# LordTARN1SHED/Image-Restoration-for-Road-Sign-Recognition-in-Autonomous-Driving

Measured on AMD Instinct MI355X. Metric: images/sec ResUNet fwd+bwd (64x64 GTSRB batch) at 1/2/4/8 MI355X; PSNR parity, higher is better.
Workload: dtype bf16; 1 GPU; cfg3: ResUNet unified train step (dynamic distortion + ToTensor, fwd + L1 + 0.1*VGG16[:16] perceptual + bwd + AdamW), 14_train_unified_advanced.py; global_batch=512, per_gpu_batch=512, parallelism=dp1, hip_graph=True

## Files before the change

image-restoration-for-road-sign-recognition-in-autonomous-driving_amd/csrc/common.h:

```cpp
#pragma once
#include <hip/hip_runtime.h>
#include <stdint.h>
#include <stdlib.h>

#include <type_traits>

#include "../../include/roadrestore.h"

typedef __bf16 bf16x8 __attribute__((ext_vector_type(8)));
typedef float f32x4 __attribute__((ext_vector_type(4)));
typedef short s16x4 __attribute__((ext_vector_type(4)));
typedef unsigned short u16;
typedef u16 u16x4 __attribute__((ext_vector_type(4)));
typedef u16 u16x8 __attribute__((ext_vector_type(8)));

#define LDS_PTR(p) ((__attribute__((address_space(3))) void *)(p))

struct bf16_t {
  u16 v;
};

__device__ __forceinline__ float bf16_to_f32(u16 b) {
  return __uint_as_float(((uint32_t)b) << 16);
}
__device__ __forceinline__ u16 f32_to_bf16(float f) {
  return __builtin_bit_cast(u16, static_cast<__bf16>(f));
}

template <typename T> struct Elt;
template <> struct Elt<float> {
  static constexpr int size = 4;
  static constexpr int dtype = RR_F32;
  __device__ __forceinline__ static float load(const float *p, long long i) { return p[i]; }
  __device__ __forceinline__ static void store(float *p, long long i, float v) { p[i] = v; }
  __device__ __forceinline__ static float round(float v) { return v; }
};
template <> struct Elt<bf16_t> {
  static constexpr int size = 2;
  static constexpr int dtype = RR_BF16;
  __device__ __forceinline__ static float load(const bf16_t *p, long long i) {
    return bf16_to_f32(p[i].v);
  }
  __device__ __forceinline__ static void store(bf16_t *p, long long i, float v) {
    p[i].v = f32_to_bf16(v);
  }
  __device__ __forceinline__ static float round(float v) { return bf16_to_f32(f32_to_bf16(v)); }
};

template <typename T> __device__ __forceinline__ f32x4 load4(const T *p);
template <> __device__ __forceinline__ f32x4 load4<float>(const float *p) {
  return *reinterpret_cast<const f32x4 *>(p);
}
template <> __device__ __forceinline__ f32x4 load4<bf16_t>(const bf16_t *p) {
  u16x4 r = *reinterpret_cast<const u16x4 *>(p);
  f32x4 o;
  o[0] = bf16_to_f32(r[0]); o[1] = bf16_to_f32(r[1]);
  o[2] = bf16_to_f32(r[2]); o[3] = bf16_to_f32(r[3]);
  return o;
}
template <typename T> __device__ __forceinline__ void store4(T *p, f32x4 v);
template <> __device__ __forceinline__ void store4<float>(float *p, f32x4 v) {
  *reinterpret_cast<f32x4 *>(p) = v;
}
template <> __device__ __forceinline__ void store4<bf16_t>(bf16_t *p, f32x4 v) {
  u16x4 r;
  r[0] = f32_to_bf16(v[0]); r[1] = f32_to_bf16(v[1]);
  r[2] = f32_to_bf16(v[2]); r[3] = f32_to_bf16(v[3]);
  *reinterpret_cast<u16x4 *>(p) = r;
}

template <typename T> __device__ __forceinline__ void load8(const T *p, f32x4 &a, f32x4 &b);
template <> __device__ __forceinline__ void load8<float>(const float *p, f32x4 &a, f32x4 &b) {
  a = *reinterpret_cast<const f32x4 *>(p);
  b = *reinterpret_cast<const f32x4 *>(p + 4);
}
template <> __device__ __forceinline__ void load8<bf16_t>(const bf16_t *p, f32x4 &a, f32x4 &b) {
  const uint4 r = *reinterpret_cast<const uint4 *>(p);
  a[0] = __uint_as_float(r.x << 16); a[1] = __uint_as_float(r.x & 0xffff0000u);
  a[2] = __uint_as_float(r.y << 16); a[3] = __uint_as_float(r.y & 0xffff0000u);
  b[0] = __uint_as_float(r.z << 16); b[1] = __uint_as_float(r.z & 0xffff0000u);
  b[2] = __uint_as_float(r.w << 16); b[3] = __uint_as_float(r.w & 0xffff0000u);
}

template <typename T> __device__ __forceinline__ void store8(T *p, f32x4 a, f32x4 b);
template <> __device__ __forceinline__ void store8<float>(float *p, f32x4 a, f32x4 b) {
  *reinterpret_cast<f32x4 *>(p) = a;
  *reinterpret_cast<f32x4 *>(p + 4) = b;
}
template <> __device__ __forceinline__ void store8<bf16_t>(bf16_t *p, f32x4 a, f32x4 b) {
  u16x8 r;
  r[0] = f32_to_bf16(a[0]); r[1] = f32_to_bf16(a[1]); r[2] = f32_to_bf16(a[2]); r[3] = f32_to_bf16(a[3]);
  r[4] = f32_to_bf16(b[0]); r[5] = f32_to_bf16(b[1]); r[6] = f32_to_bf16(b[2]); r[7] = f32_to_bf16(b[3]);
  *reinterpret_cast<u16x8 *>(p) = r;
}

template <int CTRL> __device__ __forceinline__ float dpp_f(float v) {
  return __int_as_float(__builtin_amdgcn_update_dpp(0, __float_as_int(v), CTRL, 0xF, 0xF, false));
}
constexpr int DPP_XOR1 = 0xB1, DPP_XOR2 = 0x4E, DPP_HALF_MIRROR = 0x141, DPP_MIRROR = 0x140;
__device__ __forceinline__ float row16_sum(float v) {
  v += dpp_f<DPP_XOR1>(v);
  v += dpp_f<DPP_XOR2>(v);
  v += dpp_f<DPP_HALF_MIRROR>(v);
  v += dpp_f<DPP_MIRROR>(v);
  return v;
}
__device__ __forceinline__ float max_xor1(float v) { return fmaxf(v, dpp_f<DPP_XOR1>(v)); }
__device__ __forceinline__ uint32_t xor1_u32(uint32_t v) {
  return (uint32_t)__builtin_amdgcn_update_dpp(0, (int)v, DPP_XOR1, 0xF, 0xF, false);
}
__device__ __forceinline__ float pool4_first_max(float v0, float v1, float v2, float v3, uint32_t &id) {
  float m = v0;
  uint32_t k = 0;
  bool t = !(v1 <= m) & (m == m);
  m = t ? v1 : m; k = t ? 1u : k;
  t = !(v2 <= m) & (m == m);
  m = t ? v2 : m; k = t ? 2u : k;
  t = !(v3 <= m) & (m == m);
  m = t ? v3 : m; k = t ? 3u : k;
  id = k;
  return m;
}

__device__ __forceinline__ float wave_sum(float v) {
#pragma unroll
  for (int o = 32; o > 0; o >>= 1) v += __shfl_xor(v, o, 64);
  return v;
}

#ifdef RR_DRYRUN
extern "C" void rr_dry_launch(const void *kernel, const unsigned *grid3, const unsigned *block3);
template <typename... A> static inline void rr_dry(const void *k, dim3 g, dim3 b, const A &...) {
  const unsigned g3[3] = {g.x, g.y, g.z}, b3[3] = {b.x, b.y, b.z};
  rr_dry_launch(k, g3, b3);
}
#undef hipLaunchKernelGGL
#define hipLaunchKernelGGL(k, g, b, shmem, st, ...) rr_dry((const void *)(k), dim3(g), dim3(b), __VA_ARGS__)
#define RR_LAUNCH_FAILED() false
#else
#define RR_LAUNCH_FAILED() (hipGetLastError() != hipSuccess)
#endif

#define RR_CHECK_LAUNCH()                        \
  do {                                           \
    if (RR_LAUNCH_FAILED()) return RR_ELAUNCH;   \
  } while (0)

static inline bool rr_dtype_ok(int dtype) { return dtype == RR_BF16 || dtype == RR_F32; }
template <int N> using ic = std::integral_constant<int, N>;
template <typename T> struct EltTag { using type = T; };
template <typename F> static inline int rr_dispatch_elt(int dtype, F &&f) {
  if (dtype == RR_BF16) return f(EltTag<bf16_t>{});
  if (dtype == RR_F32) return f(EltTag<float>{});
  return RR_EINVAL;
}
template <int... Vs, typename F> static inline int rr_dispatch_int(int v, F &&f) {
  int r = RR_EINVAL;
  (void)(... || (v == Vs && ((r = f(ic<Vs>{})), true)));
  return r;
}

struct RrPath {
  int stream3 = 1, stream3_strips = 1, stream1 = 1, stream1_minp = 131072;
  int conv3r = 1, conv3r_w64 = 1, conv3r_wg = 0, conv3r_segwg = 0;
  int igemm_halo = 1, swgrad = 1, wgrad_halo = 1, blur_tiled = 1;
  int rdist_tile = 32;
};

static inline RrPath rr_path_read() {
  RrPath r;
  const char *e = getenv("RR_PATH");
  if (!e || !*e) return r;
  static const struct { const char *key; int RrPath::*field; } keys[] = {
      {"stream3", &RrPath::stream3}, {"stream3_strips", &RrPath::stream3_strips},
      {"stream1", &RrPath::stream1}, {"stream1_minp", &RrPath::stream1_minp},
      {"conv3r", &RrPath::conv3r}, {"conv3r_w64", &RrPath::conv3r_w64},
      {"conv3r_wg", &RrPath::conv3r_wg}, {"conv3r_segwg", &RrPath::conv3r_segwg},
      {"igemm_halo", &RrPath::igemm_halo}, {"swgrad", &RrPath::swgrad},
      {"wgrad_halo", &RrPath::wgrad_halo}, {"blur_tiled", &RrPath::blur_tiled},
      {"rdist_tile", &RrPath::rdist_tile}};
  unsigned seen = 0;
  for (const char *p = e; *p;) {
    const char *q = p;
    while (*q && *q != ',') ++q;
    const char *eq = p;
    while (eq < q && *eq != '=') ++eq;
    const char *k0 = p, *k1 = eq, *v0 = eq < q ? eq + 1 : q, *v1 = q;
    while (k0 < k1 && *k0 == ' ') ++k0;
    while (k1 > k0 && k1[-1] == ' ') --k1;
    while (v0 < v1 && *v0 == ' ') ++v0;
    while (v1 > v0 && v1[-1] == ' ') --v1;
    const bool neg = v0 < v1 && *v0 == '-';
    if (v0 < v1 && (*v0 == '-' || *v0 == '+')) ++v0;
    int val = 0;
    bool ok = eq < q && v1 > v0 && v1 - v0 <= 9;
    for (const char *c = v0; ok && c < v1; ++c) {
      ok = *c >= '0' && *c <= '9';
      val = val * 10 + (*c - '0');
    }
    for (unsigned i = 0; ok && i < sizeof keys / sizeof keys[0]; ++i) {
      const size_t kl = __builtin_strlen(keys[i].key);
      if ((size_t)(k1 - k0) != kl || __builtin_memcmp(k0, keys[i].key, kl) != 0) continue;
      if (!(seen >> i & 1)) r.*keys[i].field = neg ? -val : val;
      seen |= 1u << i;
    }
    p = *q ? q + 1 : q;
  }
  return r;
}

static inline int rr_grid_cap(long long want, int cap = 2048) {
  if (want < 1) return 1;
  return (int)(want < cap ? want : cap);
}

static __device__ __attribute__((aligned(16))) const char rr_zero_page[256] = {0};

struct FastDiv {
  uint32_t d, m, s;
};
static inline FastDiv make_fastdiv(uint32_t d) {
  FastDiv f;
  f.d = d;
  uint32_t s = 0;
  while ((1ull << s) < d) ++s;
  f.s = s;
  f.m = (uint32_t)(((1ull << 32) * ((1ull << s) - d)) / d + 1);
  return f;
}
__device__ __forceinline__ uint32_t fdiv(uint32_t n, const FastDiv &f) {
  const uint32_t t = __umulhi(n, f.m);
  return (t + n) >> f.s;
}

template <int NC, int U = (NC == 1 ? 16 : 8), typename T>
__device__ __forceinline__ void rr_fixed_sum(const T *__restrict__ p, long long stride, long long n,
                                             double (&s)[NC]) {
  long long i = 0;
  for (; i + U <= n; i += U) {
    T v[U][NC];
#pragma unroll
    for (int u = 0; u < U; ++u)
#pragma unroll
      for (int k = 0; k < NC; ++k) v[u][k] = p[(i + u) * stride + k];
#pragma unroll
    for (int u = 0; u < U; ++u)
#pragma unroll
      for (int k = 0; k < NC; ++k) s[k] += (double)v[u][k];
  }
  for (; i < n; ++i)
#pragma unroll
    for (int k = 0; k < NC; ++k) s[k] += (double)p[i * stride + k];
}
__device__ __forceinline__ long long rr_trips(long long first, long long end, long long step) {
  return first < end ? (end - first + step - 1) / step : 0;
}

__global__ static void rr_colreduce_kernel(const float *__restrict__ in, int rows, int cols,
                                           int rows_per_chunk, double *__restrict__ out) {
  __shared__ double red[4][64];
  const int tc = threadIdx.x & 63, l = threadIdx.x >> 6;
  const int c = blockIdx.x * 64 + tc;
  const long long r0 = (long long)blockIdx.y * rows_per_chunk;
  const long long r1 = min((long long)rows, r0 + rows_per_chunk);
  double s[1] = {0.0};
  if (c < cols) rr_fixed_sum<1>(in + (r0 + l) * cols + c, 4LL * cols, rr_trips(r0 + l, r1, 4), s);
  red[l][tc] = s[0];
  __syncthreads();
  if (l == 0 && c < cols) out[(long long)blockIdx.y * cols + c] = red[0][tc] + red[1][tc] + red[2][tc] + red[3][tc];
}

static inline int rr_colreduce_chunks(int rows) { return rows < 64 ? (rows < 1 ? 1 : rows) : 64; }
static inline size_t rr_colreduce_bytes(int rows, int cols) {
  return (size_t)rr_colreduce_chunks(rows) * cols * sizeof(double);
}
static inline int rr_colreduce(const float *in, int rows, int cols, double *out, hipStream_t st) {
  const int chunks = rr_colreduce_chunks(rows);
  const int rpc = (rows + chunks - 1) / chunks;
  hipLaunchKernelGGL(rr_colreduce_kernel, dim3((cols + 63) / 64, chunks), dim3(256), 0, st, in, rows,
                     cols, rpc, out);
  return RR_LAUNCH_FAILED() ? -1 : chunks;
}
```

image-restoration-for-road-sign-recognition-in-autonomous-driving_amd/csrc/conv_in.hip:

```cpp
#include "common.h"

namespace {

template <typename T>
__global__ void conv_in_fwd_kernel(int n, int h, int w, int cin, int cout,
                                   const float *__restrict__ x, const float *__restrict__ wt,
                                   const float *__restrict__ b, int act, const float *alpha,
                                   T *__restrict__ y) {
  extern __shared__ __attribute__((aligned(16))) float sw[];
  const int kk = cin * 9;
  for (int i = threadIdx.x; i < kk * cout; i += blockDim.x) {
    const int co = i % cout, j = i / cout;
    sw[i] = wt[(long long)co * kk + j];
  }
  for (int i = threadIdx.x; i < cout; i += blockDim.x) sw[kk * cout + i] = b ? b[i] : 0.f;
  __syncthreads();
  const int G = cout / 4;
  const long long P = (long long)n * h * w;
  const float al = alpha ? alpha[0] : 0.f;
  for (long long id = blockIdx.x * (long long)blockDim.x + threadIdx.x; id < P * G;
       id += (long long)gridDim.x * blockDim.x) {
    const int g = (int)(id % G);
    const long long p = id / G;
    const int ww = (int)(p % w);
    const long long nh = p / w;
    const int hh = (int)(nh % h);
    const int nn = (int)(nh / h);
    f32x4 acc = *reinterpret_cast<const f32x4 *>(sw + kk * cout + g * 4);
    for (int ci = 0; ci < cin; ++ci) {
      const float *xp = x + ((long long)nn * cin + ci) * h * w;
#pragma unroll
      for (int t = 0; t < 9; ++t) {
        const int y2 = hh + t / 3 - 1, x2 = ww + t % 3 - 1;
        if (y2 < 0 || y2 >= h || x2 < 0 || x2 >= w) continue;
        const float v = xp[(long long)y2 * w + x2];
        acc += v * *reinterpret_cast<const f32x4 *>(sw + (ci * 9 + t) * cout + g * 4);
      }
    }
    if (act == 1) {
#pragma unroll
      for (int k = 0; k < 4; ++k) acc[k] = fmaxf(acc[k], 0.f);
    } else if (act == 2) {
#pragma unroll
      for (int k = 0; k < 4; ++k) acc[k] = acc[k] > 0.f ? acc[k] : al * acc[k];
    }
    store4<T>(y + p * cout + g * 4, acc);
  }
}

template <typename T>
__global__ void conv_in_wgrad_kernel(int n, int h, int w, int cin, int cout,
                                     const float *__restrict__ x, const T *__restrict__ dy,
                                     float *__restrict__ part, long long px_per_block) {
  __shared__ __attribute__((aligned(16))) float sdy[64][65];
  __shared__ __attribute__((aligned(16))) float spt[64][32];
  const int kk = cin * 9;
  const long long P = (long long)n * h * w;
  const long long pb = blockIdx.x * px_per_block;
  const long long pe = min(P, pb + px_per_block);
  const int co = threadIdx.x & 63, jg = threadIdx.x >> 6;
  double acc[8] = {0, 0, 0, 0, 0, 0, 0, 0};
  for (long long p0 = pb; p0 < pe; p0 += 64) {
    __syncthreads();
    for (int i = threadIdx.x; i < 64 * 64; i += blockDim.x) {
      const int r = i >> 6, c = i & 63;
      const long long p = p0 + r;
      sdy[r][c] = (p < pe && c < cout) ? Elt<T>::load(dy, p * cout + c) : 0.f;
    }
    for (int i = threadIdx.x; i < 64 * 32; i += blockDim.x) {
      const int r = i >> 5, j = i & 31;
      const long long p = p0 + r;
      float v = 0.f;
      if (p < pe) {
        if (j < kk) {
          const int ci = j / 9, t = j % 9;
          const int ww = (int)(p % w);
          const long long nh = p / w;
          const int hh = (int)(nh % h);
          const int nn = (int)(nh / h);
          const int y2 = hh + t / 3 - 1, x2 = ww + t % 3 - 1;
          if (y2 >= 0 && y2 < h && x2 >= 0 && x2 < w)
            v = x[(((long long)nn * cin + ci) * h + y2) * w + x2];
        } else if (j == kk) {
          v = 1.f;
        }
      }
      spt[r][j] = v;
    }
    __syncthreads();
    if (co < cout) {
      float st[8] = {0.f, 0.f, 0.f, 0.f, 0.f, 0.f, 0.f, 0.f};
#pragma unroll 4
      for (int r = 0; r < 64; ++r) {
        const float d = sdy[r][co];
        const f32x4 a0 = *reinterpret_cast<const f32x4 *>(&spt[r][jg * 8]);
        const f32x4 a1 = *reinterpret_cast<const f32x4 *>(&spt[r][jg * 8 + 4]);
#pragma unroll
        for (int k = 0; k < 4; ++k) { st[k] += d * a0[k]; st[4 + k] += d * a1[k]; }
      }
#pragma unroll
      for (int k = 0; k < 8; ++k) acc[k] += st[k];
    }
  }
  if (co < cout) {
#pragma unroll
    for (int k = 0; k < 8; ++k) part[((long long)blockIdx.x * cout + co) * 32 + jg * 8 + k] = (float)acc[k];
  }
}

constexpr int CIA_NPX = 64;
constexpr int CIA_ROW = CIA_NPX + 8;
constexpr int CIA_XROW = 32 + 8;
template <bool REC>
__global__ __launch_bounds__(256, REC ? 4 : 1) void conv_in_wgrad_act_kernel(
    int n, int h, int w, const float *__restrict__ x, const bf16_t *__restrict__ g,
    const bf16_t *__restrict__ t, int act, const float *__restrict__ alpha,
    float *__restrict__ part, long long ppb) {
  __shared__ __attribute__((aligned(16))) u16 gT[64 * CIA_ROW];
  __shared__ __attribute__((aligned(16))) u16 pT[32 * CIA_ROW];
  __shared__ __attribute__((aligned(16))) u16 pX[REC ? CIA_NPX * CIA_XROW : 8];
  __shared__ float red[256];
  const int tid = threadIdx.x, lane = tid & 63, wv = tid >> 6;
  const long long P = (long long)n * h * w, hw = (long long)h * w;
  const long long p0 = blockIdx.x * ppb, p1 = min(P, p0 + ppb);
  const float al = act == 2 ? alpha[0] : 0.f;
  float sa = 0.f;
  f32x4 acc[2] = {f32x4{0.f, 0.f, 0.f, 0.f}, f32x4{0.f, 0.f, 0.f, 0.f}};
  const int lc = tid & 7, lpp = tid >> 3;
  const int bn = lane & 15, bk = lane >> 4;
  const int sj = tid & 63, sg = tid >> 6;
  uint4 rg[2], rt[2] = {};
  float rp[8];
  auto load_step = [&](long long q0) __attribute__((always_inline)) {
#pragma unroll
    for (int j = 0; j < 2; ++j) {
      const long long p = q0 + 2 * lpp + j;
      const bool ok = p < p1;
      const long long e = (ok ? p : p0) * 64 + lc * 8;
      rg[j] = *reinterpret_cast<const uint4 *>(g + e);
      if constexpr (!REC) rt[j] = *reinterpret_cast<const uint4 *>(t + e);
      if (!ok) rg[j] = uint4{0u, 0u, 0u, 0u};
    }
    const long long p = q0 + sj;
    const bool live = p < p1;
    int img = 0, y = 0, xx0 = 0;
    if (live) {
      img = (int)(p / hw);
      const int rem = (int)(p - img * hw);
      y = rem / w;
      xx0 = rem - y * w;
    }
#pragma unroll
    for (int u = 0; u < 8; ++u) {
      const int r = sg + 4 * u;
      float val = 0.f;
      if (r < 27) {
        const int ci = r / 9, ky = (r % 9) / 3, kx = r % 3;
        const int yy = y + ky - 1, xx = xx0 + kx - 1;
        const bool ok = live && yy >= 0 && yy < h && xx >= 0 && xx < w;
        const float vv = x[ok ? (((long long)img * 3 + ci) * h + yy) * w + xx : 0];
        val = ok ? vv : 0.f;
      } else if (r == 27) {
        val = live ? 1.f : 0.f;
      }
      rp[u] = val;
    }
  };
  auto bf = [](uint32_t word, int hi) { return __uint_as_float(hi ? (word & 0xffff0000u) : (word << 16)); };
  bf16x8 fw = {};
  if constexpr (REC) fw = *reinterpret_cast<const bf16x8 *>(t + (wv * 16 + bn) * 32 + bk * 8);
  if (p0 < p1) load_step(p0);
  for (long long q0 = p0; q0 < p1; q0 += CIA_NPX) {
    if constexpr (REC) {
#pragma unroll
      for (int u = 0; u < 8; ++u) {
        const u16 pv = f32_to_bf16(rp[u]);
        pT[(sg + 4 * u) * CIA_ROW + sj] = pv;
        pX[sj * CIA_XROW + sg + 4 * u] = pv;
      }
      __syncthreads();
#pragma unroll
      for (int nb = 0; nb < 4; ++nb) {
        const bf16x8 fp = *reinterpret_cast<const bf16x8 *>(&pX[(nb * 16 + bn) * CIA_XROW + bk * 8]);
        const f32x4 tv = __builtin_amdgcn_mfma_f32_16x16x32_bf16(fw, fp, f32x4{0.f, 0.f, 0.f, 0.f}, 0, 0, 0);
#pragma unroll
        for (int i = 0; i < 4; ++i) gT[(wv * 16 + 4 * bk + i) * CIA_ROW + nb * 16 + bn] = f32_to_bf16(tv[i]);
      }
      __syncthreads();
    }
    u16 v[2][8];
    uint32_t tpair[8];
    if constexpr (REC) {
#pragma unroll
      for (int k = 0; k < 8; ++k)
        tpair[k] = *reinterpret_cast<const uint32_t *>(&gT[(lc * 8 + k) * CIA_ROW + 2 * lpp]);
    }
#pragma unroll
    for (int j = 0; j < 2; ++j) {
      const uint32_t gw[4] = {rg[j].x, rg[j].y, rg[j].z, rg[j].w};
      const uint32_t tw[4] = {rt[j].x, rt[j].y, rt[j].z, rt[j].w};
#pragma unroll
      for (int k = 0; k < 8; ++k) {
        const float gg = bf(gw[k >> 1], k & 1);
        const float tt = REC ? bf(tpair[k], j) : bf(tw[k >> 1], k & 1);
        const float gp = tt > 0.f ? gg : al * gg;
        sa += tt > 0.f ? 0.f : gg * tt;
        v[j][k] = f32_to_bf16(gp);
      }
    }
#pragma unroll
    for (int k = 0; k < 8; ++k)
      *reinterpret_cast<uint32_t *>(&gT[(lc * 8 + k) * CIA_ROW + 2 * lpp]) =
          (uint32_t)v[0][k] | ((uint32_t)v[1][k] << 16);
    if constexpr (!REC) {
#pragma unroll
      for (int u = 0; u < 8; ++u) pT[(sg + 4 * u) * CIA_ROW + sj] = f32_to_bf16(rp[u]);
    }
    __syncthreads();
    if (q0 + CIA_NPX < p1) load_step(q0 + CIA_NPX);
#pragma unroll
    for (int ks = 0; ks < 2; ++ks) {
      const int px = ks * 32 + bk * 8;
      const bf16x8 fa = *reinterpret_cast<const bf16x8 *>(&gT[(wv * 16 + bn) * CIA_ROW + px]);
#pragma unroll
      for (int nb = 0; nb < 2; ++nb) {
        const bf16x8 fb = *reinterpret_cast<const bf16x8 *>(&pT[(nb * 16 + bn) * CIA_ROW + px]);
        acc[nb] = __builtin_amdgcn_mfma_f32_16x16x32_bf16(fa, fb, acc[nb], 0, 0, 0);
      }
    }
    __syncthreads();
  }
  float *pw = part + (long long)blockIdx.x * (64 * 32 + 32);
#pragma unroll
  for (int nb = 0; nb < 2; ++nb)
#pragma unroll
    for (int i = 0; i < 4; ++i) pw[(wv * 16 + 4 * bk + i) * 32 + nb * 16 + bn] = acc[nb][i];
  red[tid] = sa;
  __syncthreads();
  for (int o = 128; o > 0; o >>= 1) {
    if (tid < o) red[tid] += red[tid + o];
    __syncthreads();
  }
  if (tid < 32) pw[64 * 32 + tid] = tid == 0 ? red[0] : 0.f;
}

__global__ void conv_in_wgrad_act_finalize(int chunks, const double *__restrict__ part, float *dw,
                                           float *db, float *dalpha) {
  const int i = blockIdx.x * blockDim.x + threadIdx.x;
  const int cols = 64 * 32 + 32;
  if (i > 64 * 32) return;
  double sv[1] = {0};
  rr_fixed_sum<1>(part + i, cols, chunks, sv);
  const double s = sv[0];
  if (i == 64 * 32) {
    if (dalpha) dalpha[0] = (float)s;
    return;
  }
  const int co = i / 32, j = i % 32;
  if (j < 27) dw[co * 27 + j] = (float)s;
  else if (j == 27 && db) db[co] = (float)s;
}

__global__ void conv_in_wgrad_finalize(int cout, int kk, int blocks, const double *__restrict__ part,
                                       float *dw, float *db) {
  const int i = blockIdx.x * blockDim.x + threadIdx.x;
  if (i >= cout * 32) return;
  const int co = i / 32, j = i % 32;
  if (j > kk) return;
  double sv[1] = {0};
  rr_fixed_sum<1>(part + i, (long long)cout * 32, blocks, sv);
  const double s = sv[0];
  if (j < kk) dw[(long long)co * kk + j] = (float)s;
  else if (db) db[co] = (float)s;
}

template <typename T>
__global__ void conv_in_dgrad_kernel(int n, int h, int w, int cin, int cout,
                                     const T *__restrict__ dy, const float *__restrict__ wt,
                                     float *__restrict__ dx, int accumulate) {
  extern __shared__ __attribute__((aligned(16))) float sw[];
  const int kk = cin * 9;
  for (int i = threadIdx.x; i < kk * cout; i += blockDim.x) {
    const int co = i % cout, j = i / cout;
    const int t = j / cin, ci = j % cin;
    sw[i] = wt[((long long)co * cin + ci) * 9 + t];
  }
  __syncthreads();
  const long long P = (long long)n * h * w;
  for (long long p = blockIdx.x * (long long)blockDim.x + threadIdx.x; p < P;
       p += (long long)gridDim.x * blockDim.x) {
    const int ww = (int)(p % w);
    const long long nh = p / w;
    const int hh = (int)(nh % h);
    const int nn = (int)(nh / h);
    float acc[4] = {0.f, 0.f, 0.f, 0.f};
    for (int t = 0; t < 9; ++t) {
      const int ky = t / 3, kx = t % 3;
      const int y2 = hh - ky + 1, x2 = ww - kx + 1;
      if (y2 < 0 || y2 >= h || x2 < 0 || x2 >= w) continue;
      const T *dp = dy + (((long long)nn * h + y2) * w + x2) * cout;
      for (int c = 0; c < cout; c += 4) {
        const f32x4 d = load4<T>(dp + c);
        for (int ci = 0; ci < cin && ci < 4; ++ci) {
          const f32x4 wv = *reinterpret_cast<const f32x4 *>(sw + (t * cin + ci) * cout + c);
          acc[ci] += d[0] * wv[0] + d[1] * wv[1] + d[2] * wv[2] + d[3] * wv[3];
        }
      }
    }
    for (int ci = 0; ci < cin && ci < 4; ++ci) {
      const long long o = (((long long)nn * cin + ci) * h + hh) * w + ww;
      dx[o] = accumulate ? dx[o] + acc[ci] : acc[ci];
    }
  }
}

template <typename T>
__global__ void im2col3_kernel(int n, int h, int w, int cin, int kpad, const float *__restrict__ x,
                               T *__restrict__ col) {
  const int G = kpad / 4;
  const long long total = (long long)n * h * w * G;
  const int kk = cin * 9;
  for (long long i = blockIdx.x * (long long)blockDim.x + threadIdx.x; i < total;
       i += (long long)gridDim.x * blockDim.x) {
    const int g = (int)(i % G);
    const long long p = i / G;
    const int ww = (int)(p % w);
    const long long nh = p / w;
    const int hh = (int)(nh % h);
    const int nn = (int)(nh / h);
    f32x4 v;
#pragma unroll
    for (int e = 0; e < 4; ++e) {
      const int j = g * 4 + e;
      float val = 0.f;
      if (j < kk) {
        const int ci = j / 9, t = j - (j / 9) * 9;
        const int y2 = hh + t / 3 - 1, x2 = ww + t % 3 - 1;
        if (y2 >= 0 && y2 < h && x2 >= 0 && x2 < w)
          val = x[(((long long)nn * cin + ci) * h + y2) * w + x2];
      } else if (j == kk) {
        val = 1.f;
      }
      v[e] = val;
    }
    store4<T>(col + p * kpad + g * 4, v);
  }
}

__global__ __launch_bounds__(256) void conv_in_mfma_kernel(int n, int h, int w,
                                                           const float *__restrict__ x,
                                                           const bf16_t *__restrict__ wp, int act,
                                                           const float *__restrict__ alpha,
                                                           bf16_t *__restrict__ y_pre,
                                                           bf16_t *__restrict__ y_act) {
  constexpr int SR = 68;
  __shared__ __attribute__((aligned(16))) float stg[4][32 * SR];
  const int lane = threadIdx.x & 63, wv = threadIdx.x >> 6;
  const long long hw = (long long)h * w;
  const long long P = (long long)n * hw;
  const long long p0 = ((long long)blockIdx.x * 4 + wv) * 64;
  if (p0 >= P) return;
  const int fr = lane & 15, q = lane >> 4;
  bf16x8 fa[4];
#pragma unroll
  for (int mi = 0; mi < 4; ++mi)
    fa[mi] = *reinterpret_cast<const bf16x8 *>(wp + (mi * 16 + fr) * 32 + q * 8);
  const int hwi = h * w;
  int kofs[8], kdy[8], kdx[8];
  bool ktap[8], kone[8];
#pragma unroll
  for (int j = 0; j < 8; ++j) {
    const int k = q * 8 + j;
    const int ci = k / 9, t = k - (k / 9) * 9;
    kdy[j] = t / 3 - 1;
    kdx[j] = t % 3 - 1;
    kofs[j] = ci * hwi + kdy[j] * w + kdx[j];
    ktap[j] = k < 27;
    kone[j] = k == 27;
  }
  const int Pi = (int)P;
  const __amdgpu_buffer_rsrc_t xr = __builtin_amdgcn_make_buffer_rsrc(
      const_cast<float *>(x), 0, (int)(3 * P * 4), 0x00020000);
  const int pw0 = (int)p0;
  f32x4 acc[4][4];
#pragma unroll
  for (int ni = 0; ni < 4; ++ni) {
    const int p = pw0 + ni * 16 + fr;
    const bool live = p < Pi;
    const int pc = live ? p : 0;
    const int nn = pc / hwi, rem = pc - (pc / hwi) * hwi;
    const int yy = rem / w, xx = rem - (rem / w) * w;
    const int base = nn * 3 * hwi + rem;
    bf16x8 fb;
#pragma unroll
    for (int j = 0; j < 8; ++j) {
      const int y2 = yy + kdy[j], x2 = xx + kdx[j];
      const bool ok = ktap[j] && live && (unsigned)y2 < (unsigned)h && (unsigned)x2 < (unsigned)w;
      const float v = __builtin_bit_cast(float, __builtin_amdgcn_raw_buffer_load_b32(
          xr, ok ? (base + kofs[j]) * 4 : 0xffffffff, 0, 0));
      fb[j] = (__bf16)(v + (kone[j] ? 1.f : 0.f));
    }
#pragma unroll
    for (int mi = 0; mi < 4; ++mi)
      acc[mi][ni] = __builtin_amdgcn_mfma_f32_16x16x32_bf16(fa[mi], fb, f32x4{0.f, 0.f, 0.f, 0.f},
                                                           0, 0, 0);
  }
  float *sw = stg[wv];
  const float slope = act == 2 ? alpha[0] : (act == 1 ? 0.f : 1.f);
  const int rows = (int)min(64LL, P - p0);
#pragma unroll
  for (int half = 0; half < 2; ++half) {
    if (half) asm volatile("s_waitcnt lgkmcnt(0)" ::: "memory");
#pragma unroll
    for (int mi = 0; mi < 4; ++mi)
#pragma unroll
      for (int nj = 0; nj < 2; ++nj)
        *reinterpret_cast<f32x4 *>(sw + (nj * 16 + fr) * SR + mi * 16 + q * 4) = acc[mi][half * 2 + nj];
    asm volatile("s_waitcnt lgkmcnt(0)" ::: "memory");
#pragma unroll
    for (int i = 0; i < 4; ++i) {
      const int rl = i * 8 + (lane >> 3), c8 = (lane & 7) * 8;
      const int r = half * 32 + rl;
      if (r < rows) {
        const long long p = p0 + r;
        const f32x4 v0 = *reinterpret_cast<const f32x4 *>(sw + rl * SR + c8);
        const f32x4 v1 = *reinterpret_cast<const f32x4 *>(sw + rl * SR + c8 + 4);
        if (y_pre) store8<bf16_t>(y_pre + p * 64 + c8, v0, v1);
        if (y_act) {
          f32x4 a0, a1;
#pragma unroll
          for (int k = 0; k < 4; ++k) {
            a0[k] = v0[k] > 0.f ? v0[k] : slope * v0[k];
            a1[k] = v1[k] > 0.f ? v1[k] : slope * v1[k];
          }
          store8<bf16_t>(y_act + p * 64 + c8, a0, a1);
        }
      }
    }
  }
}

}

extern "C" int rr_im2col3(int dtype, int n, int h, int w, int cin, int kpad, const float *x,
                          void *col, rr_stream stream) {
  if (!x || !col || cin <= 0 || kpad % 4 || kpad < 9 * cin + 1) return RR_EINVAL;
  const long long total = (long long)n * h * w * (kpad / 4);
  dim3 g(rr_grid_cap((total + 255) / 256, 8192)), b(256);
  hipStream_t st = (hipStream_t)stream;
  return rr_dispatch_elt(dtype, [&](auto tag) {
    using T = typename decltype(tag)::type;
    hipLaunchKernelGGL(im2col3_kernel<T>, g, b, 0, st, n, h, w, cin, kpad, x, (T *)col);
    RR_CHECK_LAUNCH();
    return RR_OK;
  });
}

extern "C" int rr_conv_in_fwd(int dtype, int n, int h, int w, int cin, int cout, const float *x,
                              const float *wt, const float *b, int act, const float *alpha,
                              void *y, rr_stream stream) {
  if (!x || !wt || !y || n <= 0 || h <= 0 || w <= 0 || cin <= 0 || cin > 4 || cout % 4 ||
      cout > 128 || (act == 2 && !alpha))
    return RR_EINVAL;
  const long long work = (long long)n * h * w * (cout / 4);
  const size_t shm = ((size_t)cin * 9 * cout + cout) * sizeof(float);
  dim3 g(rr_grid_cap((work + 255) / 256, 8192)), bl(256);
  hipStream_t st = (hipStream_t)stream;
  return rr_dispatch_elt(dtype, [&](auto tag) {
    using T = typename decltype(tag)::type;
    hipLaunchKernelGGL(conv_in_fwd_kernel<T>, g, bl, shm, st, n, h, w, cin, cout, x, wt, b, act,
                       alpha, (T *)y);
    RR_CHECK_LAUNCH();
    return RR_OK;
  });
}

int rr_colreduce_misc(const float *in, int rows, int cols, double *out, hipStream_t st);
static int conv_in_wgrad_blocks(int n, int h, int w) {
  const long long P = (long long)n * h * w;
  long long b = (P + 2047) / 2048;
  if (b > 1024) b = 1024;
  return (int)(b < 1 ? 1 : b);
}

extern "C" size_t rr_conv_in_wgrad_workspace(int n, int h, int w, int cin, int cout) {
  (void)cin;
  const int blocks = conv_in_wgrad_blocks(n, h, w);
  return (size_t)blocks * cout * 32 * sizeof(float) + rr_colreduce_bytes(blocks, cout * 32);
}

extern "C" int rr_conv_in_wgrad(int dtype, int n, int h, int w, int cin, int cout, const float *x,
                                const void *dy, float *dw, float *db, void *ws, size_t ws_bytes,
                                rr_stream stream) {
  if (!x || !dy || !dw || cin * 9 >= 32 || cout > 64 || cout <= 0) return RR_EINVAL;
  const int blocks = conv_in_wgrad_blocks(n, h, w);
  const size_t pbytes = (size_t)blocks * cout * 32 * sizeof(float);
  if (!ws || ws_bytes < pbytes + rr_colreduce_bytes(blocks, cout * 32)) return RR_EWORKSPACE;
  const long long P = (long long)n * h * w;
  long long ppb = (P + blocks - 1) / blocks;
  hipStream_t st = (hipStream_t)stream;
  const int rc = rr_dispatch_elt(dtype, [&](auto tag) {
    using T = typename decltype(tag)::type;
    hipLaunchKernelGGL(conv_in_wgrad_kernel<T>, dim3(blocks), dim3(256), 0, st, n, h, w, cin, cout,
                       x, (const T *)dy, (float *)ws, ppb);
    RR_CHECK_LAUNCH();
    return RR_OK;
  });
  if (rc != RR_OK) return rc;
  double *red = (double *)((char *)ws + pbytes);
  const int chunks = rr_colreduce_misc((const float *)ws, blocks, cout * 32, red, st);
  if (chunks < 0) return RR_ELAUNCH;
  hipLaunchKernelGGL(conv_in_wgrad_finalize, dim3((cout * 32 + 255) / 256), dim3(256), 0, st, cout,
                     cin * 9, chunks, (const double *)red, dw, db);
  RR_CHECK_LAUNCH();
  return RR_OK;
}

static int conv_in_act_blocks(long long P) {
  long long b = (P + 511) / 512;
  if (b > 2048) b = 2048;
  return (int)(b < 1 ? 1 : b);
}

extern "C" size_t rr_conv_in_wgrad_act_workspace(int n, int h, int w) {
  const int blocks = conv_in_act_blocks((long long)n * h * w);
  return (size_t)blocks * (64 * 32 + 32) * sizeof(float) + rr_colreduce_bytes(blocks, 64 * 32 + 32);
}

static int conv_in_wgrad_act(bool rec, int n, int h, int w, const float *x, const void *dy,
                             const void *t_pre, int act, const float *alpha, float *dw, float *db,
                             float *dalpha, void *ws, size_t ws_bytes, rr_stream stream) {
  if (!x || !dy || !t_pre || !dw || n <= 0 || h <= 0 || w <= 0) return RR_EINVAL;
  if (act < 1 || act > 2 || (act == 2 && !alpha)) return RR_EINVAL;
  const long long P = (long long)n * h * w;
  const int blocks = conv_in_act_blocks(P);
  const size_t pbytes = (size_t)blocks * (64 * 32 + 32) * sizeof(float);
  if (!ws || ws_bytes < pbytes + rr_colreduce_bytes(blocks, 64 * 32 + 32)) return RR_EWORKSPACE;
  long long ppb = (P + blocks - 1) / blocks;
  ppb = (ppb + CIA_NPX - 1) / CIA_NPX * CIA_NPX;
  hipStream_t st = (hipStream_t)stream;
  if (rec)
    hipLaunchKernelGGL(conv_in_wgrad_act_kernel<true>, dim3(blocks), dim3(256), 0, st, n, h, w, x,
                       (const bf16_t *)dy, (const bf16_t *)t_pre, act, alpha, (float *)ws, ppb);
  else
    hipLaunchKernelGGL(conv_in_wgrad_act_kernel<false>, dim3(blocks), dim3(256), 0, st, n, h, w, x,
                       (const bf16_t *)dy, (const bf16_t *)t_pre, act, alpha, (float *)ws, ppb);
  RR_CHECK_LAUNCH();
  double *red = (double *)((char *)ws + pbytes);
  const int chunks = rr_colreduce_misc((const float *)ws, blocks, 64 * 32 + 32, red, st);
  if (chunks < 0) return RR_ELAUNCH;
  hipLaunchKernelGGL(conv_in_wgrad_act_finalize, dim3((64 * 32 + 1 + 255) / 256), dim3(256), 0, st,
                     chunks, (const double *)red, dw, db, act == 2 ? dalpha : nullptr);
  RR_CHECK_LAUNCH();
  return RR_OK;
}

extern "C" int rr_conv_in_wgrad_act(int n, int h, int w, const float *x, const void *dy,
                                    const void *t_pre, int act, const float *alpha, float *dw,
                                    float *db, float *dalpha, void *ws, size_t ws_bytes,
                                    rr_stream stream) {
  return conv_in_wgrad_act(false, n, h, w, x, dy, t_pre, act, alpha, dw, db, dalpha, ws, ws_bytes, stream);
}

extern "C" int rr_conv_in_wgrad_act_rec(int n, int h, int w, const float *x, const void *dy,
                                        const void *wpack32, int act, const float *alpha, float *dw,
                                        float *db, float *dalpha, void *ws, size_t ws_bytes,
                                        rr_stream stream) {
  return conv_in_wgrad_act(true, n, h, w, x, dy, wpack32, act, alpha, dw, db, dalpha, ws, ws_bytes, stream);
}

extern "C" int rr_conv_in_dgrad(int dtype, int n, int h, int w, int cin, int cout, const void *dy,
                                const float *wt, float *dx, int accumulate, rr_stream stream) {
  if (!dy || !wt || !dx || cin > 4 || cout % 4) return RR_EINVAL;
  const long long P = (long long)n * h * w;
  const size_t shm = (size_t)cin * 9 * cout * sizeof(float);
  dim3 g(rr_grid_cap((P + 255) / 256, 8192)), b(256);
  hipStream_t st = (hipStream_t)stream;
  return rr_dispatch_elt(dtype, [&](auto tag) {
    using T = typename decltype(tag)::type;
    hipLaunchKernelGGL(conv_in_dgrad_kernel<T>, g, b, shm, st, n, h, w, cin, cout, (const T *)dy, wt,
                       dx, accumulate);
    RR_CHECK_LAUNCH();
    return RR_OK;
  });
}

extern "C" int rr_conv_in_mfma(int n, int h, int w, const float *x, const void *wpack32, int act,
                               const float *alpha, void *y_pre, void *y_act, rr_stream stream) {
  if (!x || !wpack32 || (!y_pre && !y_act) || n <= 0 || h <= 0 || w <= 0) return RR_EINVAL;
  if (act < 0 || act > 2 || (act == 2 && !alpha) || (y_act == nullptr && act != 0)) return RR_EINVAL;
  const long long P = (long long)n * h * w;
  if (12 * P >= 0x7fffffffLL) return RR_EUNSUPPORTED;
  const long long blocks = (P + 255) / 256;
  hipLaunchKernelGGL(conv_in_mfma_kernel, dim3((unsigned)blocks), dim3(256), 0, (hipStream_t)stream,
                     n, h, w, x, (const bf16_t *)wpack32, act, alpha, (bf16_t *)y_pre,
                     (bf16_t *)y_act);
  RR_CHECK_LAUNCH();
  return RR_OK;
}
```

Baseline: 36910 images/sec.

## Add row-tiled first-layer conv wgrad kernel with LDS halo tile and double staging

Adds a new weight-gradient kernel for the first 3-input-channel conv layer with fused activation backward. It loads a halo tile of input rows into LDS once and builds the im2col patches from it, instead of gathering each tap separately. It also processes NS slices per iteration, with register prefetch of the next rows and gradients, and XOR-swizzles the gradient tile. The aim is to cut redundant global gathers and overlap loads with MFMA work. The cost is more LDS and register use, and a new path that only applies when width and h*w meet divisibility conditions; it is on by default via the first_fast flag.

Measured after the change: 37150 images/sec, median of 6. No clear change (+0.6%).

```diff
diff --git a/image-restoration-for-road-sign-recognition-in-autonomous-driving_amd/csrc/common.h b/image-restoration-for-road-sign-recognition-in-autonomous-driving_amd/csrc/common.h
--- a/image-restoration-for-road-sign-recognition-in-autonomous-driving_amd/csrc/common.h
+++ b/image-restoration-for-road-sign-recognition-in-autonomous-driving_amd/csrc/common.h
@@ -165,6 +165,7 @@
   int conv3r = 1, conv3r_w64 = 1, conv3r_wg = 0, conv3r_segwg = 0;
   int igemm_halo = 1, swgrad = 1, wgrad_halo = 1, blur_tiled = 1;
   int rdist_tile = 32;
+  int first_fast = 1;
 };
 
 static inline RrPath rr_path_read() {
@@ -178,7 +179,7 @@
       {"conv3r_wg", &RrPath::conv3r_wg}, {"conv3r_segwg", &RrPath::conv3r_segwg},
       {"igemm_halo", &RrPath::igemm_halo}, {"swgrad", &RrPath::swgrad},
       {"wgrad_halo", &RrPath::wgrad_halo}, {"blur_tiled", &RrPath::blur_tiled},
-      {"rdist_tile", &RrPath::rdist_tile}};
+      {"rdist_tile", &RrPath::rdist_tile}, {"first_fast", &RrPath::first_fast}};
   unsigned seen = 0;
   for (const char *p = e; *p;) {
     const char *q = p;
diff --git a/image-restoration-for-road-sign-recognition-in-autonomous-driving_amd/csrc/conv_in.hip b/image-restoration-for-road-sign-recognition-in-autonomous-driving_amd/csrc/conv_in.hip
--- a/image-restoration-for-road-sign-recognition-in-autonomous-driving_amd/csrc/conv_in.hip
+++ b/image-restoration-for-road-sign-recognition-in-autonomous-driving_amd/csrc/conv_in.hip
@@ -235,6 +235,219 @@
   for (int nb = 0; nb < 2; ++nb)
 #pragma unroll
     for (int i = 0; i < 4; ++i) pw[(wv * 16 + 4 * bk + i) * 32 + nb * 16 + bn] = acc[nb][i];
+  red[tid] = sa;
+  __syncthreads();
+  for (int o = 128; o > 0; o >>= 1) {
+    if (tid < o) red[tid] += red[tid + o];
+    __syncthreads();
+  }
+  if (tid < 32) pw[64 * 32 + tid] = tid == 0 ? red[0] : 0.f;
+}
+
+constexpr int CIF_TILE = 600;
+template <bool REC, int NS>
+__global__ __launch_bounds__(256, 4) void conv_in_wgrad_act_rows_kernel(
+    int n, int h, int w, int lw, const float *__restrict__ x, const bf16_t *__restrict__ g,
+    const bf16_t *__restrict__ t, int act, const float *__restrict__ alpha,
+    float *__restrict__ part, long long ppb) {
+  __shared__ __attribute__((aligned(16))) u16 gT[NS][64 * CIA_ROW];
+  __shared__ __attribute__((aligned(16))) u16 pT[NS][32 * CIA_ROW];
+  __shared__ __attribute__((aligned(16))) u16 pX[REC ? NS : 1][REC ? CIA_NPX * CIA_XROW : 8];
+  __shared__ __attribute__((aligned(16))) u16 tl[NS][CIF_TILE];
+  const int tid = threadIdx.x, lane = tid & 63, wv = tid >> 6;
+  const int hw = h * w;
+  const long long P = (long long)n * hw;
+  const long long p0 = blockIdx.x * ppb, p1 = min(P, p0 + ppb);
+  const float al = act == 2 ? alpha[0] : 0.f;
+  float sa = 0.f;
+  f32x4 acc[2] = {f32x4{0.f, 0.f, 0.f, 0.f}, f32x4{0.f, 0.f, 0.f, 0.f}};
+  const int lc = tid & 7, lpp = tid >> 3;
+  const int bn = lane & 15, bk = lane >> 4;
+  const int twi = 1 << lw, rs = 64 >> lw, tw = twi + 2, plane = (rs + 2) * tw, ne = 3 * plane;
+  int eo[4], er[4], ec[4];
+#pragma unroll
+  for (int u = 0; u < 4; ++u) {
+    const int e = 2 * (tid + 256 * (u >> 1)) + (u & 1);
+    const int e2 = e < ne ? e : 0;
+    const int ci = e2 / plane, rr = (e2 - ci * plane) / tw, c = e2 - ci * plane - rr * tw;
+    er[u] = e < ne ? rr - 1 : -1 - h;
+    ec[u] = c - 1;
+    eo[u] = ci * hw + (rr - 1) * w + (c - 1);
+  }
+  auto tap = [&](int k, int px) {
+    const int ci = k / 9, ky = (k % 9) / 3, kx = k % 3;
+    return ci * plane + ((px >> lw) + ky) * tw + (px & (twi - 1)) + kx;
+  };
+  const int tr = tid >> 3, tg = tid & 7;
+  const int xp = tid >> 2, xg = tid & 3;
+  int po[8], xo[8];
+#pragma unroll
+  for (int j = 0; j < 8; ++j) {
+    po[j] = tap(tr < 27 ? tr : 0, tg * 8 + j);
+    xo[j] = tap(xg * 8 + j < 27 ? xg * 8 + j : 0, xp);
+  }
+  for (int i = tid; i < NS * 5 * 32; i += 256) {
+    const int s = i / 160, r = (i % 160) / 32, c2 = i % 32;
+    *reinterpret_cast<uint32_t *>(&pT[s][(27 + r) * CIA_ROW + 2 * c2]) = r == 0 ? 0x3f803f80u : 0u;
+  }
+  long long cb = 0;
+  int cy = 0, cx = 0;
+  if (p0 < p1) {
+    const long long img = p0 / hw;
+    const int rem = (int)(p0 - img * hw);
+    cb = img * 3 * hw;
+    cy = rem / w;
+    cx = rem - cy * w;
+  }
+  uint4 rg[NS][2], rt[NS][2] = {};
+  float ri[NS][4];
+  auto load_rows = [&](long long q0) __attribute__((always_inline)) {
+#pragma unroll
+    for (int s = 0; s < NS; ++s) {
+      if (q0 + s * CIA_NPX >= p1) break;
+      const int at = cy * w + cx;
+#pragma unroll
+      for (int u = 0; u < 4; ++u) {
+        const int yy = cy + er[u], xx = cx + ec[u];
+        const bool ok = (unsigned)yy < (unsigned)h && (unsigned)xx < (unsigned)w;
+        const float vv = x[ok ? cb + (at + eo[u]) : 0];
+        ri[s][u] = ok ? vv : 0.f;
+      }
+      cx += CIA_NPX;
+      if (cx >= w) { cx = 0; cy += rs; }
+      if (cy >= h) { cy = 0; cb += 3LL * hw; }
+    }
+  };
+  auto store_rows = [&](long long q0) __attribute__((always_inline)) {
+#pragma unroll
+    for (int s = 0; s < NS; ++s) {
+      if (q0 + s * CIA_NPX >= p1) break;
+#pragma unroll
+      for (int v = 0; v < 2; ++v) {
+        const int e = 2 * (tid + 256 * v);
+        if (e < ne)
+          *reinterpret_cast<uint32_t *>(&tl[s][e]) =
+              (uint32_t)f32_to_bf16(ri[s][2 * v]) | ((uint32_t)f32_to_bf16(ri[s][2 * v + 1]) << 16);
+      }
+    }
+  };
+  auto load_g = [&](long long q0) __attribute__((always_inline)) {
+#pragma unroll
+    for (int s = 0; s < NS; ++s) {
+      if (q0 + s * CIA_NPX >= p1) break;
+#pragma unroll
+      for (int j = 0; j < 2; ++j) {
+        const long long e = (q0 + s * CIA_NPX + 2 * lpp + j) * 64 + lc * 8;
+        rg[s][j] = *reinterpret_cast<const uint4 *>(g + e);
+        if constexpr (!REC) rt[s][j] = *reinterpret_cast<const uint4 *>(t + e);
+      }
+    }
+  };
+  auto gi = [](int row, int px) { return row * CIA_ROW + (px ^ (((row >> 3) & 7) << 3)); };
+  auto bf = [](uint32_t word, int hi) { return __uint_as_float(hi ? (word & 0xffff0000u) : (word << 16)); };
+  bf16x8 fw = {};
+  if constexpr (REC) fw = *reinterpret_cast<const bf16x8 *>(t + (wv * 16 + bn) * 32 + bk * 8);
+  if (p0 < p1) {
+    load_rows(p0);
+    load_g(p0);
+    store_rows(p0);
+  }
+  __syncthreads();
+  for (long long q0 = p0; q0 < p1; q0 += NS * CIA_NPX) {
+    const long long qn = q0 + NS * CIA_NPX;
+    if (qn < p1) load_rows(qn);
+#pragma unroll
+    for (int s = 0; s < NS; ++s) {
+      if (q0 + s * CIA_NPX >= p1) break;
+      if (tr < 27) {
+        uint32_t pk[4];
+#pragma unroll
+        for (int j = 0; j < 4; ++j)
+          pk[j] = (uint32_t)tl[s][po[2 * j]] | ((uint32_t)tl[s][po[2 * j + 1]] << 16);
+        *reinterpret_cast<uint4 *>(&pT[s][tr * CIA_ROW + tg * 8]) = uint4{pk[0], pk[1], pk[2], pk[3]};
+      }
+      if constexpr (REC) {
+        u16 pv[8];
+#pragma unroll
+        for (int j = 0; j < 8; ++j) {
+          const int k = xg * 8 + j;
+          const u16 tv = tl[s][xo[j]];
+          pv[j] = k < 27 ? tv : (u16)(k == 27 ? 0x3f80 : 0);
+        }
+        *reinterpret_cast<uint4 *>(&pX[s][xp * CIA_XROW + xg * 8]) =
+            uint4{(uint32_t)pv[0] | ((uint32_t)pv[1] << 16), (uint32_t)pv[2] | ((uint32_t)pv[3] << 16),
+                  (uint32_t)pv[4] | ((uint32_t)pv[5] << 16), (uint32_t)pv[6] | ((uint32_t)pv[7] << 16)};
+      }
+    }
+    if constexpr (REC) {
+      __syncthreads();
+#pragma unroll
+      for (int s = 0; s < NS; ++s) {
+        if (q0 + s * CIA_NPX >= p1) break;
+#pragma unroll
+        for (int nb = 0; nb < 4; ++nb) {
+          const bf16x8 fp = *reinterpret_cast<const bf16x8 *>(&pX[s][(nb * 16 + bn) * CIA_XROW + bk * 8]);
+          const f32x4 tv = __builtin_amdgcn_mfma_f32_16x16x32_bf16(fp, fw, f32x4{0.f, 0.f, 0.f, 0.f}, 0, 0, 0);
+          *reinterpret_cast<uint2 *>(&gT[s][gi(wv * 16 + bn, nb * 16 + 4 * bk)]) =
+              uint2{(uint32_t)f32_to_bf16(tv[0]) | ((uint32_t)f32_to_bf16(tv[1]) << 16),
+                    (uint32_t)f32_to_bf16(tv[2]) | ((uint32_t)f32_to_bf16(tv[3]) << 16)};
+        }
+      }
+      __syncthreads();
+    }
+#pragma unroll
+    for (int s = 0; s < NS; ++s) {
+      if (q0 + s * CIA_NPX >= p1) break;
+      u16 v[2][8];
+      uint32_t tpair[8];
+      if constexpr (REC) {
+#pragma unroll
+        for (int k = 0; k < 8; ++k)
+          tpair[k] = *reinterpret_cast<const uint32_t *>(&gT[s][gi(lc * 8 + k, 2 * lpp)]);
+      }
+#pragma unroll
+      for (int j = 0; j < 2; ++j) {
+        const uint32_t gw[4] = {rg[s][j].x, rg[s][j].y, rg[s][j].z, rg[s][j].w};
+        const uint32_t tw4[4] = {rt[s][j].x, rt[s][j].y, rt[s][j].z, rt[s][j].w};
+#pragma unroll
+        for (int k = 0; k < 8; ++k) {
+          const float gg = bf(gw[k >> 1], k & 1);
+          const float tt = REC ? bf(tpair[k], j) : bf(tw4[k >> 1], k & 1);
+          const float gp = tt > 0.f ? gg : al * gg;
+          sa += tt > 0.f ? 0.f : gg * tt;
+          v[j][k] = f32_to_bf16(gp);
+        }
+      }
+#pragma unroll
+      for (int k = 0; k < 8; ++k)
+        *reinterpret_cast<uint32_t *>(&gT[s][gi(lc * 8 + k, 2 * lpp)]) =
+            (uint32_t)v[0][k] | ((uint32_t)v[1][k] << 16);
+    }
+    if (qn < p1) load_g(qn);
+    __syncthreads();
+#pragma unroll
+    for (int s = 0; s < NS; ++s) {
+      if (q0 + s * CIA_NPX >= p1) break;
+#pragma unroll
+      for (int ks = 0; ks < 2; ++ks) {
+        const int px = ks * 32 + bk * 8;
+        const bf16x8 fa = *reinterpret_cast<const bf16x8 *>(&gT[s][gi(wv * 16 + bn, px)]);
+#pragma unroll
+        for (int nb = 0; nb < 2; ++nb) {
+          const bf16x8 fb = *reinterpret_cast<const bf16x8 *>(&pT[s][(nb * 16 + bn) * CIA_ROW + px]);
+          acc[nb] = __builtin_amdgcn_mfma_f32_16x16x32_bf16(fa, fb, acc[nb], 0, 0, 0);
+        }
+      }
+    }
+    if (qn < p1) store_rows(qn);
+    __syncthreads();
+  }
+  float *pw = part + (long long)blockIdx.x * (64 * 32 + 32);
+#pragma unroll
+  for (int nb = 0; nb < 2; ++nb)
+#pragma unroll
+    for (int i = 0; i < 4; ++i) pw[(wv * 16 + 4 * bk + i) * 32 + nb * 16 + bn] = acc[nb][i];
+  float *red = reinterpret_cast<float *>(&gT[0][0]);
   red[tid] = sa;
   __syncthreads();
   for (int o = 128; o > 0; o >>= 1) {
@@ -527,7 +740,7 @@
   return (size_t)blocks * (64 * 32 + 32) * sizeof(float) + rr_colreduce_bytes(blocks, 64 * 32 + 32);
 }
 
-static int conv_in_wgrad_act(bool rec, int n, int h, int w, const float *x, const void *dy,
+static int conv_in_wgrad_act(bool rec, int first_fast, int n, int h, int w, const float *x, const void *dy,
                              const void *t_pre, int act, const float *alpha, float *dw, float *db,
                              float *dalpha, void *ws, size_t ws_bytes, rr_stream stream) {
   if (!x || !dy || !t_pre || !dw || n <= 0 || h <= 0 || w <= 0) return RR_EINVAL;
@@ -539,7 +752,23 @@
   long long ppb = (P + blocks - 1) / blocks;
   ppb = (ppb + CIA_NPX - 1) / CIA_NPX * CIA_NPX;
   hipStream_t st = (hipStream_t)stream;
-  if (rec)
+  const long long hw = (long long)h * w;
+  const bool rows = first_fast != 0 && (64 % w == 0 || w % 64 == 0) && hw % 64 == 0 && 3 * hw < 0x7fffffffLL;
+  if (rows) {
+    int lw = 0;
+    while ((2 << lw) <= (w < 64 ? w : 64)) ++lw;
+    const auto launch = [&](auto kernel) {
+      hipLaunchKernelGGL(kernel, dim3(blocks), dim3(256), 0, st, n, h, w, lw, x, (const bf16_t *)dy,
+                         (const bf16_t *)t_pre, act, alpha, (float *)ws, ppb);
+    };
+    if (first_fast == 64) {
+      if (rec) launch(conv_in_wgrad_act_rows_kernel<true, 1>);
+      else launch(conv_in_wgrad_act_rows_kernel<false, 1>);
+    } else {
+      if (rec) launch(conv_in_wgrad_act_rows_kernel<true, 2>);
+      else launch(conv_in_wgrad_act_rows_kernel<false, 2>);
+    }
+  } else if (rec)
     hipLaunchKernelGGL(conv_in_wgrad_act_kernel<true>, dim3(blocks), dim3(256), 0, st, n, h, w, x,
                        (const bf16_t *)dy, (const bf16_t *)t_pre, act, alpha, (float *)ws, ppb);
   else
@@ -559,14 +788,14 @@
                                     const void *t_pre, int act, const float *alpha, float *dw,
                                     float *db, float *dalpha, void *ws, size_t ws_bytes,
                                     rr_stream stream) {
-  return conv_in_wgrad_act(false, n, h, w, x, dy, t_pre, act, alpha, dw, db, dalpha, ws, ws_bytes, stream);
+  return conv_in_wgrad_act(false, rr_path_read().first_fast, n, h, w, x, dy, t_pre, act, alpha, dw, db, dalpha, ws, ws_bytes, stream);
 }
 
 extern "C" int rr_conv_in_wgrad_act_rec(int n, int h, int w, const float *x, const void *dy,
                                         const void *wpack32, int act, const float *alpha, float *dw,
                                         float *db, float *dalpha, void *ws, size_t ws_bytes,
                                         rr_stream stream) {
-  return conv_in_wgrad_act(true, n, h, w, x, dy, wpack32, act, alpha, dw, db, dalpha, ws, ws_bytes, stream);
+  return conv_in_wgrad_act(true, rr_path_read().first_fast, n, h, w, x, dy, wpack32, act, alpha, dw, db, dalpha, ws, ws_bytes, stream);
 }
 
 extern "C" int rr_conv_in_dgrad(int dtype, int n, int h, int w, int cin, int cout, const void *dy,
```
